# fabrizioromanelli/ORBSLAM2

Hardware: AMD Instinct MI355X
Metric: frames/sec ORB extract+match, KITTI 1241×376 stereo, 2000 feats; 1/2/4/8 GPU (higher is better)
Workload: dtype u8; 1 GPU; Stereo-KITTI00-02 1241x376, 2000 features, 8 levels: extract L+R + ComputeStereoMatches (64 pairs per step per GPU, weak scaling); distinct_pairs=16, chains_in_flight=1, stream_groups=1, quadtree_kernel=3, parallelism=frame-pair sharding, no data-path collective

## Files before the change

### orbslam2_amd/csrc/orbfe_api.hip

```cpp
#include "orbfe_host.h"

#include <algorithm>
#include <chrono>
#include <cmath>
#include <cstdarg>
#include <cstdio>
#include <cstdlib>
#include <cstring>
#include <new>
#include <vector>

static const int8_t k_bit_pattern_31[1024] = {
#include "orb_pattern_31.inc"
};
static thread_local char g_err[512] = "";

int orbfe_fail(orbfe_context *ctx, int code, const char *fmt, ...)
{
    char msg[512];
    va_list ap;
    va_start(ap, fmt);
    vsnprintf(msg, sizeof(msg), fmt, ap);
    va_end(ap);
    snprintf(g_err, sizeof(g_err), "%s", msg);
// ... 161 lines not shown
    T(&b.tail_plan, P.tail_plan, "pyramid tail plan");
    T(&b.pair_plan, P.pair_plan, "pyramid pair plan");
    T(&b.rs_tab, P.rs_tab, "resize table");
    T(&b.cell_aux, P.cell_aux, "cell table");
    T(&b.fast_lane_tab, P.fast_lane_tab, "cell table");
    T(&b.cell_info, P.cell_info, "cell table");
    T(&b.bk_tab, P.bk_tab, "bucket table");
    T(&b.bk_off, P.bk_off, "bucket partial table");
    T(&b.bk_emap, P.bk_emap, "bucket partial table");
    A(b.bk_part, B * P.bk_emap.size());
    T(&b.blur_tile_info, P.blur_tile_info, "blur tile table");
    T(&b.slot_level, P.slot_level, "slot table");
    T(&b.patch_uv, P.patch_uv, "patch table");
    T(&b.mom_tab, P.mom_tab, "moment table");
    uint32_t *d_pat = nullptr;
    A(d_pat, 256);
    if (rc == ORBFE_OK && hipMemcpy(d_pat, k_bit_pattern_31, 1024, hipMemcpyHostToDevice) != hipSuccess) rc = orbfe_fail(ctx, ORBFE_ERR_HIP, "pattern upload failed");
    b.pattern = d_pat;
    memcpy(ctx->pattern, k_bit_pattern_31, 1024);
    b.lv0 = b.pyr + c.lv[0].pyr_off; b.lv0_stride = c.pyr_bytes; b.lv0_pitch = c.lv[0].pitch; b.lv0_packed = 0;
    Z(b.proc_xy, B * c.sel_total * sizeof(uint32_t)); Z(b.proc_meta, B * c.sel_total * sizeof(uint32_t));
    Z(b.dbg_ts, 4096 * sizeof(long long)); Z(b.row_cnt, pairs * (size_t)p.height * sizeof(int));
    Z(b.bk_part, B * P.bk_emap.size() * sizeof(uint32_t));
    Z(b.kp_cnt, sizeof(int) * B); Z(b.sel_cnt, sizeof(int) * B * c.nlevels); Z(b.status, sizeof(int) * B);
    if (rc != ORBFE_OK) { orbfe_destroy(ctx); return rc; }
    *out = ctx;
    return ORBFE_OK;
} ORBFE_CATCH(nullptr)

extern "C" void orbfe_destroy(orbfe_context *ctx)
{
    if (!ctx) return;
    if (ctx->stream) { hipStreamSynchronize(ctx->stream); }
    for (void *q : ctx->allocs) hipFree(q);
    for (hipEvent_t e : ctx->events) hipEventDestroy(e);
    for (int g = 0; g < ORBFE_MAX_GROUPS; g++) {
        if (ctx->gstreams[g]) { hipStreamSynchronize(ctx->gstreams[g]); hipStreamDestroy(ctx->gstreams[g]); }
        if (ctx->ev_join[g]) hipEventDestroy(ctx->ev_join[g]);
    }
    if (ctx->ev_fork) hipEventDestroy(ctx->ev_fork);
    if (ctx->ev_latest) hipEventDestroy(ctx->ev_latest);
    if (ctx->ev_pack) { if (ctx->ev_pack_set) hipEventSynchronize(ctx->ev_pack); hipEventDestroy(ctx->ev_pack); }
    if (ctx->match) orbfe_match_state_destroy(ctx->match);
    if (ctx->match_device) orbfe_match_device_state_destroy(ctx->match_device);
    if (ctx->bow) orbfe_bow_state_destroy(ctx->bow);
    if (ctx->pose) orbfe_pose_state_destroy(ctx->pose);
    if (ctx->d_depth_in) hipFree(ctx->d_depth_in);
    if (ctx->h_in) hipHostFree(ctx->h_in);
    if (ctx->h_depth_in) hipHostFree(ctx->h_depth_in);
    if (ctx->h_out) hipHostFree(ctx->h_out);
    for (int sd = 0; sd < 2; sd++) { if (ctx->cfg.rm_xy[sd]) hipFree((void *)ctx->cfg.rm_xy[sd]); if (ctx->cfg.rm_a[sd]) hipFree((void *)ctx->cfg.rm_a[sd]); }
    if (ctx->stream) hipStreamDestroy(ctx->stream);
    delete ctx;
}

extern "C" int orbfe_get_camera(const orbfe_context *ctx, float *cam)
try {
    if (!ctx || !cam) return ORBFE_ERR_INVALID;
    cam[0] = ctx->params.fx; cam[1] = ctx->params.fy; cam[2] = ctx->params.cx; cam[3] = ctx->params.cy; cam[4] = ctx->params.bf;
    return ORBFE_OK;
} ORBFE_CATCH(nullptr)

static int wait_latest(orbfe_context *ctx);
extern "C" int orbfe_set_pattern(orbfe_context *ctx, const int32_t *pattern)
try {
    ORBFE_ENTRY(ctx);
// ... 125 lines not shown
    const size_t i = (size_t)img0;
    o.pyr += i * c.pyr_bytes; o.blur += i * c.blur_bytes;
    o.lv0 = o.pyr + c.lv[0].pyr_off; o.lv0_stride = c.pyr_bytes; o.lv0_pitch = c.lv[0].pitch; o.lv0_packed = 0;
    o.cell_cnt += i * c.cells_total; o.cell_base += i * c.cells_total;
    o.cell_xy += i * c.cells_total * c.cell_cap; o.cell_sc += i * c.cells_total * c.cell_cap;
    o.cand_xy += i * c.cand_total; o.cand_sc += i * c.cand_total;
    o.idx0 += i * c.cand_total; o.idx1 += i * c.cand_total; o.ot_xy2 += i * c.cand_total;
    o.lvl_ncand += i * c.nlevels; o.sel_cnt += i * c.nlevels;
    o.bk_part += i * c.bk_part_total; o.bk_end += i * c.nlevels * 4097;
    if (o.ot3_scratch) o.ot3_scratch += i * c.nlevels * orbfe_octree3_node_bytes(c.max_nodes, orbfe_sort_cap(c.max_nodes));
    if (o.bk_best) o.bk_best += i * c.nlevels * ORBFE_BK_PYR;
    if (o.otg_scratch) o.otg_scratch += i * orbfe_otg_level_off(c, c.nlevels);
    o.sel_xy += i * c.sel_total; o.sel_sc += i * c.sel_total; o.proc_xy += i * c.sel_total; o.proc_meta += i * c.sel_total;
    o.kps = (KeyPointPOD *)o.kps + i * c.sel_total; o.desc += i * c.sel_total * 32;
    o.kp_cnt += i; o.status += i;
    o.u_right += i * c.sel_total; o.depth += i * c.sel_total; o.sad += i * c.sel_total;
    o.row_cnt += (i / 2) * (size_t)c.height; o.row_ent += (i / 2) * (size_t)c.height * c.row_cap;
    return o;
}

static int blur_ride_from_of(const orbfe_context *ctx, int n_images)
{
    if (!ctx->plan.fuse_blur) return ctx->cfg.nlevels;
    return n_images >= ctx->plan.blur_ride_min_images ? (ctx->plan.blur_ride_from < ctx->cfg.nlevels ? ctx->plan.blur_ride_from : ctx->cfg.nlevels) : ORBFE_MAX_LEVELS;
}

extern "C" int orbfe_blur_ride_from(const orbfe_context *ctx, int n_images)
try {
    if (!ctx) return ORBFE_ERR_INVALID;
    const int r = blur_ride_from_of(ctx, n_images);
    return r < ctx->cfg.nlevels ? r : (ctx->plan.fuse_blur && n_images < ctx->plan.blur_ride_min_images ? ctx->cfg.nlevels - 1 : ctx->cfg.nlevels);
} ORBFE_CATCH(nullptr)

static void run_chain(orbfe_context *ctx, const uint8_t *d_images, int img0, int n_images, int n_pairs, hipStream_t s, int group)
{
    const DeviceConfig &cfg = ctx->cfg;
    DeviceBuffers buf = shift_buffers(ctx->buf, cfg, img0);
    const uint8_t *src = d_images + (size_t)img0 * cfg.in_image_bytes;
    prof_mark(ctx, group, 0, s);
    if (ctx->plan.inplace_ok && cfg.in_cn == 1 && !cfg.rm_on) {
        buf.lv0 = src; buf.lv0_stride = cfg.in_image_bytes; buf.lv0_pitch = cfg.width; buf.lv0_packed = 1;
    } else {
        orbfe_launch_ingest(cfg, buf, src, n_images, s);
    }
    prof_mark(ctx, group, 1, s);
    const int ride_from = blur_ride_from_of(ctx, n_images);
    const int blurred = orbfe_launch_pyramid(cfg, buf, n_images, ctx->plan.fuse_blur, s, ride_from);
    prof_mark(ctx, group, 2, s);
    if (!ctx->plan.fuse_blur) orbfe_launch_blur(cfg, buf, n_images, blurred, s);
    prof_mark(ctx, group, 3, s);
    orbfe_launch_fast(cfg, buf, n_images, ctx->plan.use_octree3, s, ctx->plan.fuse_blur ? blurred : cfg.nlevels);
    prof_mark(ctx, group, 4, s);
    if (ctx->plan.use_octree3) orbfe_launch_octree3(cfg, buf, n_images, ctx->plan.ot_sort_cap, ctx->plan.ot3_lds, ctx->plan.ot3_nodes_in_hbm, s);
    else if (const hipError_t e = orbfe_launch_octree_generic(cfg, buf, n_images, ctx->plan.otg_nodes_in_hbm, s)) ctx->chain_err = e;
#ifdef ORBFE_PROFILE_CUTS
    {
        extern void orbfe_launch_dbg_sort_sel(const DeviceConfig &, const DeviceBuffers &, int, int, hipStream_t);
        static const int dbg_sort = getenv("ORBFE_DBG_SORT_SEL") ? atoi(getenv("ORBFE_DBG_SORT_SEL")) : 0;
        if (dbg_sort) orbfe_launch_dbg_sort_sel(cfg, buf, n_images, dbg_sort, s);
    }
#endif
    prof_mark(ctx, group, 5, s);
    orbfe_launch_describe(cfg, buf, n_images, n_pairs > 0, s);
    prof_mark(ctx, group, 6, s);
    if (n_pairs > 0) {
        if (cfg.half_patch != 15) orbfe_launch_stereo_rowlists(cfg, buf, n_pairs, s);
        orbfe_launch_stereo_match(cfg, buf, n_pairs, s);
        prof_mark(ctx, group, 7, s);
        orbfe_launch_stereo_median(cfg, buf, n_pairs, s);
        prof_mark(ctx, group, 8, s);
    }
}

static int enqueue_batch(orbfe_context *ctx, const uint8_t *d_images, int n_units, int imgs_per_unit, void *stream)
{
    hipStream_t s;
    if (const int rc = orbfe_enqueue_on(ctx, stream, false, &s)) return rc;
    ctx->prof_now = ctx->profiling && (ctx->prof_seq++ % (unsigned)ctx->prof_every) == 0;
    const int n_images = n_units * imgs_per_unit;
    int G = ctx->groups < n_units ? ctx->groups : n_units;
    if (G < 1) G = 1;
    if (G == 1) {
        run_chain(ctx, d_images, 0, n_images, imgs_per_unit == 2 ? n_units : 0, s, 0);
    } else {
        ORBFE_HIP_TRY(ctx, hipEventRecord(ctx->ev_fork, s));
        int u0 = 0;
        for (int g = 0; g < G; g++) {
            const int nu = n_units / G + (g < n_units % G ? 1 : 0);
            hipStream_t sg = ctx->gstreams[g];
            ORBFE_HIP_TRY(ctx, hipStreamWaitEvent(sg, ctx->ev_fork, 0));
            run_chain(ctx, d_images, u0 * imgs_per_unit, nu * imgs_per_unit, imgs_per_unit == 2 ? nu : 0, sg, g);
            ORBFE_HIP_TRY(ctx, hipEventRecord(ctx->ev_join[g], sg));
            ORBFE_HIP_TRY(ctx, hipStreamWaitEvent(s, ctx->ev_join[g], 0));
            u0 += nu;
        }
    }
    if (ctx->chain_err != hipSuccess) { const hipError_t e = ctx->chain_err; ctx->chain_err = hipSuccess; return orbfe_fail(ctx, ORBFE_ERR_HIP, "quadtree launch: %s", hipGetErrorString(e)); }
    ORBFE_HIP_TRY(ctx, hipGetLastError());
    ctx->last_src = (ctx->plan.inplace_ok && ctx->cfg.in_cn == 1 && !ctx->cfg.rm_on) ? d_images : nullptr;
    ctx->last_src_owned = ctx->last_src && ctx->last_src == ctx->d_in;
    ctx->last_images = n_images;
    ctx->epoch++;
    ctx->prof_groups = G;
    ctx->latest_foreign = s != ctx->stream;
    if (ctx->latest_foreign) ORBFE_HIP_TRY(ctx, hipEventRecord(ctx->ev_latest, s));
    if (ctx->prof_now) ctx->prof_calls++;
    return ORBFE_OK;
}

extern "C" int orbfe_quadtree_kernel(const orbfe_context *ctx)
try {
    if (!ctx) return 0;
    return ctx->plan.use_octree3 ? 3 : 1;
} ORBFE_CATCH(nullptr)

extern "C" int orbfe_quadtree_plan(const orbfe_context *ctx)
try {
    if (!ctx) return ORBFE_ERR_INVALID;
    if (ctx->plan.use_octree3) return ctx->plan.ot3_nodes_in_hbm ? 1 : 0;
    return ctx->plan.otg_nodes_in_hbm ? 3 : 2;
} ORBFE_CATCH(nullptr)

extern "C" int orbfe_set_streams(orbfe_context *ctx, int groups)
try {
    ORBFE_ENTRY(ctx);
    if (!ctx || groups < 1 || groups > ORBFE_MAX_GROUPS) return orbfe_fail(ctx, ORBFE_ERR_INVALID, "groups must be in [1, %d]", ORBFE_MAX_GROUPS);
    if (ctx->profiling) return orbfe_fail(ctx, ORBFE_ERR_INVALID, "change the stream count before enabling profiling");
    ORBFE_HIP_TRY(ctx, hipSetDevice(ctx->params.device));
    if (!ctx->ev_fork) ORBFE_HIP_TRY(ctx, hipEventCreateWithFlags(&ctx->ev_fork, hipEventDisableTiming));
    for (int g = 0; g < groups; g++) {
// ... 608 lines not shown
        return orbfe_fail(ctx, ORBFE_ERR_INVALID, "bad argument");
    { const int rcw = wait_latest(ctx); if (rcw != ORBFE_OK) return rcw; }
    const LevelInfo &L = ctx->cfg.lv[level];
    if (dst_stride < (size_t)L.w) return orbfe_fail(ctx, ORBFE_ERR_INVALID, "dst_stride smaller than level width");
    if (blurred) {
        const size_t bytes = (size_t)L.blur_tx * ((L.h + 3) / 4) * 128;
        std::vector<uint8_t> t(bytes);
        ORBFE_HIP_TRY(ctx, hipMemcpy(t.data(), ctx->buf.blur + (size_t)image * ctx->cfg.blur_bytes + L.blur_off, bytes, hipMemcpyDeviceToHost));
        for (int y = 0; y < L.h; y++)
            for (int x = 0; x < L.w; x += 4) {
                const size_t off = ((size_t)(y >> 2) * L.blur_tx + (x >> 5)) * 128 + (size_t)((x & 31) >> 2) * 16 + (size_t)(y & 3) * 4;
                memcpy(dst + (size_t)y * dst_stride + x, t.data() + off, (size_t)std::min(4, L.w - x));
            }
        return ORBFE_OK;
    }
    if (level == 0 && !blurred && ctx->last_src) {
        if (!ctx->last_src_owned && !ctx->input_retained)
            return orbfe_fail(ctx, ORBFE_ERR_UNSUPPORTED, "level 0 of the latest call is the caller's own image buffer (read in place, never copied): "
                                                    "call orbfe_set_input_retained(ctx, 1) if that buffer is still valid, or read the images there");
        ORBFE_HIP_TRY(ctx, hipMemcpy2D(dst, dst_stride, ctx->last_src + (size_t)image * ctx->cfg.in_image_bytes, (size_t)L.w, (size_t)L.w, (size_t)L.h, hipMemcpyDeviceToHost));
        return ORBFE_OK;
    }
    const uint8_t *src = ctx->buf.pyr + (size_t)image * ctx->cfg.pyr_bytes + L.pyr_off;
    ORBFE_HIP_TRY(ctx, hipMemcpy2D(dst, dst_stride, src, (size_t)L.pitch, (size_t)L.w, (size_t)L.h, hipMemcpyDeviceToHost));
    return ORBFE_OK;
} ORBFE_CATCH(ctx)

extern "C" int orbfe_fetch_candidates(orbfe_context *ctx, int image, int level, int32_t *xs, int32_t *ys,
                                      int32_t *scores, int cap, int *n)
try {
    ORBFE_ENTRY(ctx);
    if (!ctx || !n || image < 0 || image >= ctx->params.max_images || level < 0 || level >= ctx->cfg.nlevels)
        return orbfe_fail(ctx, ORBFE_ERR_INVALID, "bad argument");
    { const int rcw = wait_latest(ctx); if (rcw != ORBFE_OK) return rcw; }
    const DeviceConfig &c = ctx->cfg;
    const LevelInfo &L = c.lv[level];
    if (ctx->plan.use_octree3) {
        orbfe_launch_candidates_gather(c, ctx->buf, ctx->params.max_images, ctx->stream);
        ORBFE_HIP_TRY(ctx, hipStreamSynchronize(ctx->stream));
    }
    int nc = 0;
    ORBFE_HIP_TRY(ctx, hipMemcpy(&nc, ctx->buf.lvl_ncand + (size_t)image * c.nlevels + level, sizeof(int), hipMemcpyDeviceToHost));
    *n = nc;
    if (nc > cap) return orbfe_fail(ctx, ORBFE_ERR_CAPACITY, "caller buffers hold %d candidates, level has %d", cap, nc);
    if (nc == 0) return ORBFE_OK;
    std::vector<uint32_t> xy(nc);
    std::vector<uint8_t> sc(nc);
    ORBFE_HIP_TRY(ctx, hipMemcpy(xy.data(), ctx->buf.cand_xy + (size_t)image * c.cand_total + L.cand_off, sizeof(uint32_t) * nc, hipMemcpyDeviceToHost));
    ORBFE_HIP_TRY(ctx, hipMemcpy(sc.data(), ctx->buf.cand_sc + (size_t)image * c.cand_total + L.cand_off, (size_t)nc, hipMemcpyDeviceToHost));
    for (int i = 0; i < nc; i++) {
        if (xs) xs[i] = (int32_t)(xy[i] & 0xffffu);
        if (ys) ys[i] = (int32_t)(xy[i] >> 16);
        if (scores) scores[i] = sc[i];
    }
    return ORBFE_OK;
} ORBFE_CATCH(ctx)
```

### orbslam2_amd/csrc/orbfe_config.h

```cpp
#pragma once

#include <math.h>
#include <stddef.h>
#include <stdint.h>

#ifdef __HIPCC__
#define ORBFE_HD __attribute__((host, device)) inline __attribute__((always_inline))
#else
#define ORBFE_HD inline
#endif

#define ORBFE_MAX_LEVELS 16
#define ORBFE_TAIL_MAX 3
#define ORBFE_TAIL_COLS 64
#ifndef ORBFE_BLUR_ROWS
#define ORBFE_BLUR_ROWS 32
#endif
#define ORBFE_WAVE 64
#define PYR_MX 4
#define PYR_MY 3
#ifndef ORBFE_PYR_RB
#define ORBFE_PYR_RB 4
#endif
struct LevelInfo {
// ... 31 lines not shown
    int width, height;
    int edge_threshold, min_border;
    int ini_th, min_th;
    uint32_t ini_th_h2, min_th_h2;
    int half_patch;
    int cell_cap;
    int cells_total;
    int cand_total;
    int sel_total;
    int blur_tiles_total;
    int proc_order;
    int fast_blur_t0;
    uint32_t xcd_magic;
    int max_nodes;
    int bk_part_total;
    int row_cap;
    int patch_n;
    int tail_first, tail_n, tail_strips;
    int pp_max_images;
    int tail_max_images;
    int tail_src_words;
    int tail_words[ORBFE_TAIL_MAX];
    int tail_lds_y[ORBFE_TAIL_MAX];
    int tail_lds_buf[ORBFE_TAIL_MAX];
    int tail_lds_src, tail_lds_bytes;
    int umax[64];
    int taps[7];
    size_t pyr_bytes;
    size_t blur_bytes;
    float bf, fx, mb;
    int in_cn, in_coef[3], in_shift;
    size_t in_image_bytes;
    int rm_on, rm_sw, rm_sh;
    const uint32_t *rm_xy[2];
    const uint16_t *rm_a[2];
    int n_dist;
    float dist[5];
    float cam[4];
    LevelInfo lv[ORBFE_MAX_LEVELS];
};
static_assert(sizeof(LevelInfo) == 224 && sizeof(DeviceConfig) == 4168, "LevelInfo / DeviceConfig layout changed");
static_assert(offsetof(DeviceConfig, pyr_bytes) == 440 && offsetof(DeviceConfig, rm_xy) == 512 && offsetof(DeviceConfig, lv) == 584,
              "DeviceConfig layout changed");

#define ORBFE_BK_DEPTH 5
#define ORBFE_BK_BUCKETS 4096
#define ORBFE_BK_PYR 5460
#define ORBFE_BK_REF_MASK 0xffffffu
#define ORBFE_BK_KEY(sc, cell, slot) (((sc) << 24) | (ORBFE_BK_REF_MASK - (unsigned)(((cell) << 12) | (slot))))
#define ORBFE_BK_PART(cnt, key) ((cnt) | (((key) & 0xfffu) << 12) | ((key) & 0xff000000u))
#define ORBFE_BK_PART_KEY(e, cell) (((e) & 0xff000000u) | ((4095u - (unsigned)(cell)) << 12) | (((e) >> 12) & 0xfffu))

#define OT3_ROOTS 4
#define OT3_PYR (OT3_ROOTS * 1365)
#define OT3_HI (OT3_ROOTS * 85)

ORBFE_HD int resize_first_source(int dx, double scale, int src_w)
{
    const float fx = (float)(((double)dx + 0.5) * scale - 0.5);
    int sx = (int)floorf(fx);
    sx = sx < 0 ? 0 : sx;
    return sx >= src_w - 1 ? src_w - 1 : sx;
}
ORBFE_HD int resize_word_base(int xw, int dst_w, double scale, int src_w)
{
    int lo = 0x7fffffff;
    for (int j = 0; j < 4; j++) {
        int q = 4 * xw + j - PYR_MX;
        if (dst_w == 1) q = 0;
        else while (q < 0 || q >= dst_w) q = q < 0 ? -q : 2 * dst_w - 2 - q;
        lo = q < lo ? q : lo;
    }
    return resize_first_source(lo, scale, src_w);
}

static inline int max_cell_w(const DeviceConfig &cfg) { int m = 0; for (int l = 0; l < cfg.nlevels; l++) m = cfg.lv[l].w_cell > m ? cfg.lv[l].w_cell : m; return m; }
// ... 42 lines not shown
```

### orbslam2_amd/csrc/orbfe_device.h

```cpp
#pragma once

#include <hip/hip_runtime.h>
#include <stdint.h>
#include <stdlib.h>

#include "orbfe_config.h"

typedef unsigned long long u64;

#ifdef ORBFE_PROFILE_CUTS
#define ORBFE_CUT_PARAM , int dbg
template <int N> __device__ __forceinline__ bool orbfe_phase_end() { asm volatile("; ORBFE_PHASE_END %0" ::"n"(N)); return true; }
#define ORBFE_CUT(n) (orbfe_phase_end<n>() && dbg == (n))
#define ORBFE_CUT_ARG(env) , orbfe_cut_value(env)
static inline int orbfe_cut_value(const char *env) { const char *v = getenv(env); return v ? atoi(v) : 0; }
#else
#define ORBFE_CUT_PARAM
#define ORBFE_CUT(n) false
#define ORBFE_CUT_ARG(env)
#endif

struct DeviceBuffers {
    uint8_t *pyr;
    const uint8_t *lv0;
// ... 26 lines not shown
    int *sad;
    int *status;
    int *row_cnt;
    uint2 *row_ent;
    const uint32_t *bk_tab;
    const uint32_t *bk_emap;
    const uint32_t *bk_off;
    const uint32_t *rs_tab;
    const uint4 *cell_info;
    const uint2 *cell_aux;
    const uint32_t *fast_lane_tab;
    const uint32_t *blur_tile_info;
    const uint32_t *rs_blk;
    const int *pair_plan;
    const int *tail_plan;
    long long *dbg_ts;
    const uint8_t *slot_level;
    const int16_t *patch_uv;
    const uint32_t *mom_tab;
    const uint32_t *pattern;
    uint8_t *otg_scratch;
};

struct KeyPointPOD {
    float x, y, size, angle, response;
    int32_t octave, class_id;
};
static_assert(sizeof(KeyPointPOD) == 28, "keypoint must match cv::KeyPoint");

void orbfe_launch_ingest(const DeviceConfig &cfg, const DeviceBuffers &buf, const uint8_t *d_images,
                         int n_images, hipStream_t s);
int orbfe_launch_pyramid(const DeviceConfig &cfg, const DeviceBuffers &buf, int n_images, bool fuse_blur, hipStream_t s, int ride_from = ORBFE_MAX_LEVELS);
void orbfe_launch_blur(const DeviceConfig &cfg, const DeviceBuffers &buf, int n_images, int first_level, hipStream_t s);
void orbfe_launch_fast(const DeviceConfig &cfg, const DeviceBuffers &buf, int n_images, bool buckets, hipStream_t s, int blur_first_level);
hipError_t orbfe_launch_octree_generic(const DeviceConfig &cfg, const DeviceBuffers &buf, int n_images, bool nodes_in_hbm, hipStream_t s);
int orbfe_octree_generic_prepare(const DeviceConfig &cfg, bool nodes_in_hbm);
void orbfe_launch_octree3(const DeviceConfig &cfg, const DeviceBuffers &buf, int n_images, int sort_cap, size_t lds, bool nodes_in_hbm, hipStream_t s);
void orbfe_launch_candidates_gather(const DeviceConfig &cfg, const DeviceBuffers &buf, int n_images, hipStream_t s);
int orbfe_octree3_prepare(size_t lds, bool nodes_in_hbm);
void orbfe_launch_describe(const DeviceConfig &cfg, const DeviceBuffers &buf, int n_images, bool stereo, hipStream_t s);
void orbfe_launch_stereo_rowlists(const DeviceConfig &cfg, const DeviceBuffers &buf, int n_pairs, hipStream_t s);
void orbfe_launch_stereo_match(const DeviceConfig &cfg, const DeviceBuffers &buf, int n_pairs, hipStream_t s);
void orbfe_launch_stereo_median(const DeviceConfig &cfg, const DeviceBuffers &buf, int n_pairs, hipStream_t s);
void orbfe_launch_rgbd(const DeviceConfig &cfg, const DeviceBuffers &buf, const float *d_depth,
                       size_t depth_pitch_floats, int image, hipStream_t s);
void orbfe_launch_undistort(const DeviceConfig &cfg, const void *d_keys_in, void *d_keys_out, int n, hipStream_t s);
struct GridFrame;
void orbfe_launch_grid_build(const GridFrame &f, hipStream_t s);
struct orbfe_context;
struct orbfe_grid_keyframe;
int orbfe_grid_frame_of_record(orbfe_context *ctx, const orbfe_grid_keyframe *kf, GridFrame &f);
void orbfe_launch_rgbd_u16(const DeviceConfig &cfg, const DeviceBuffers &buf, const uint16_t *d_depth, size_t depth_pitch_px,
                           float factor, int image, hipStream_t s);
void orbfe_launch_rgbd_batch(const DeviceConfig &cfg, const DeviceBuffers &buf, const void *d_depth, bool is_u16, float factor, int n_images, hipStream_t s);
struct PackedOffsets { size_t counts, level_counts, xy, angle, response, desc, u_right, depth; };
void orbfe_launch_pack_results(const DeviceConfig &cfg, const DeviceBuffers &buf, uint8_t *d_out, const PackedOffsets &lay, int n_out, int img_step, bool stereo, hipStream_t s);
```

### orbslam2_amd/csrc/orbfe_fast.hip

```cpp
#include "orbfe_common.hpp"
#include "orbfe_blur_wave.hpp"

__device__ __forceinline__ int fast_score16(const uint8_t *t, int pitch, int minth)
{
    const int v = t[0];
    int d[16];
    d[0] = v - t[3 * pitch];       d[1] = v - t[3 * pitch + 1];   d[2] = v - t[2 * pitch + 2];   d[3] = v - t[pitch + 3];
    d[4] = v - t[3];               d[5] = v - t[-pitch + 3];      d[6] = v - t[-2 * pitch + 2];  d[7] = v - t[-3 * pitch + 1];
    d[8] = v - t[-3 * pitch];      d[9] = v - t[-3 * pitch - 1];  d[10] = v - t[-2 * pitch - 2]; d[11] = v - t[-pitch - 3];
    d[12] = v - t[-3];             d[13] = v - t[pitch - 3];      d[14] = v - t[2 * pitch - 2];  d[15] = v - t[3 * pitch - 1];
    int mn2[16], mx2[16], mn4[16], mx4[16];
#pragma unroll
    for (int k = 0; k < 16; k++) { mn2[k] = min(d[k], d[(k + 1) & 15]); mx2[k] = max(d[k], d[(k + 1) & 15]); }
#pragma unroll
    for (int k = 0; k < 16; k++) { mn4[k] = min(mn2[k], mn2[(k + 2) & 15]); mx4[k] = max(mx2[k], mx2[(k + 2) & 15]); }
    int a = -512, b = 512;
#pragma unroll
    for (int k = 0; k < 16; k++) {
        const int mn9 = min(min(mn4[k], mn4[(k + 4) & 15]), d[(k + 8) & 15]);
        const int mx9 = max(max(mx4[k], mx4[(k + 4) & 15]), d[(k + 8) & 15]);
        a = max(a, mn9);
        b = min(b, mx9);
    }
    return max(minth, max(a, -b)) - 1;
// ... 26 lines not shown
    int r;
    unsigned long long c;
    asm("v_addc_co_u32_e64 %0, %1, %2, 0, %3" : "=v"(r), "=s"(c) : "v"(x), "s"(m));
    return r;
}

__device__ __forceinline__ unsigned long long neg_lo16(unsigned v) { unsigned long long m; asm("v_cmp_gt_i16_e64 %0, 0, %1" : "=s"(m) : "v"(v)); return m; }
__device__ __forceinline__ unsigned long long neg_hi16(unsigned v) { unsigned long long m; asm("v_cmp_gt_i32_e64 %0, 0, %1" : "=s"(m) : "v"(v)); return m; }
__device__ __forceinline__ unsigned lds_addr(const void *p) { return (unsigned)(unsigned long)(__attribute__((address_space(3))) const void *)p; }
__device__ __forceinline__ void lds_store_lo16(unsigned long long m, unsigned addr, unsigned v)
{
    unsigned long long save;
    asm volatile("s_and_saveexec_b64 %0, %1\n\tds_write_b16 %2, %3\n\ts_or_b64 exec, exec, %0" : "=&s"(save) : "s"(m), "v"(addr), "v"(v) : "memory", "scc");
}
__device__ __forceinline__ void lds_store_hi16(unsigned long long m, unsigned addr, unsigned v)
{
    unsigned long long save;
    asm volatile("s_and_saveexec_b64 %0, %1\n\tds_write_b16_d16_hi %2, %3\n\ts_or_b64 exec, exec, %0" : "=&s"(save) : "s"(m), "v"(addr), "v"(v) : "memory", "scc");
}

__device__ __forceinline__ unsigned h2min(unsigned a, unsigned b) { unsigned d; asm("v_pk_min_f16 %0, %1, %2" : "=v"(d) : "v"(a), "v"(b)); return d; }
__device__ __forceinline__ unsigned h2max(unsigned a, unsigned b) { unsigned d; asm("v_pk_max_f16 %0, %1, %2" : "=v"(d) : "v"(a), "v"(b)); return d; }
__device__ __forceinline__ unsigned h2min3(unsigned a, unsigned b, unsigned c) { unsigned d; asm("v_pk_minimum3_f16 %0, %1, %2, %3" : "=v"(d) : "v"(a), "v"(b), "v"(c)); return d; }
__device__ __forceinline__ unsigned h2max3(unsigned a, unsigned b, unsigned c) { unsigned d; asm("v_pk_maximum3_f16 %0, %1, %2, %3" : "=v"(d) : "v"(a), "v"(b), "v"(c)); return d; }
__device__ __forceinline__ unsigned h2add(unsigned a, unsigned b) { unsigned d; asm("v_pk_add_f16 %0, %1, %2" : "=v"(d) : "v"(a), "v"(b)); return d; }
__device__ __forceinline__ unsigned h2sub(unsigned a, unsigned b) { unsigned d; asm("v_pk_add_f16 %0, %1, %2 neg_lo:[0,1] neg_hi:[0,1]" : "=v"(d) : "v"(a), "v"(b)); return d; }

#define FAST_WAVE_SYNC() do { __builtin_amdgcn_s_waitcnt(0xc07f); __builtin_amdgcn_wave_barrier(); } while (0)
template <int TP, bool BK>
__global__ __launch_bounds__(256) __attribute__((amdgpu_waves_per_eu(6, 8))) void fast_cell_kernel(DeviceConfig cfg, DeviceBuffers buf, int n_images, int tile_pitch_rt, int tile_bytes, int sc_bytes, int q_bytes, int lds_per_wave ORBFE_CUT_PARAM)
{
    const int tile_pitch = TP ? TP : tile_pitch_rt;
    extern __shared__ __attribute__((aligned(16))) uint8_t s_mem_all[];
    const int bpi_cells = (cfg.cells_total + 3) >> 2;
    const int bpi = bpi_cells + ((cfg.blur_tiles_total - cfg.fast_blur_t0 + 3) >> 2);
    int img, blk;
    if (!xcd_map_magic(bpi, n_images, cfg.xcd_magic, img, blk)) return;
    const int wave = __builtin_amdgcn_readfirstlane((int)(threadIdx.x >> 6));
    if (__builtin_expect(blk >= bpi_cells, 0)) {
        const int u = cfg.fast_blur_t0 + (blk - bpi_cells) * 4 + wave;
        if (u < cfg.blur_tiles_total) blur_wave(cfg, buf, img, u);
        return;
    }
    const int cell = blk * 4 + wave;
    if (cell >= cfg.cells_total) return;
    uint8_t *s_mem = s_mem_all + wave * lds_per_wave;
    const uint4 cinfo = const_load_u32x4(buf.cell_info + cell);
    const uint32_t aux_g = const_load_u32((const uint32_t *)buf.cell_aux + 2 * cell), aux_c = const_load_u32((const uint32_t *)buf.cell_aux + 2 * cell + 1);
    const uint32_t *lane_tab = buf.fast_lane_tab + ((aux_g & 0x1ffffu) << 9);
    const uint4 lt_a = *(const uint4 *)(lane_tab + ((threadIdx.x & 63) << 3));
    const uint2 lt_b = *(const uint2 *)(lane_tab + ((threadIdx.x & 63) << 3) + 4);
    const int level = (int)(cinfo.x & 0xffu);
    const LevelInfo &L = cfg.lv[level];
    const int ci = (int)cinfo.w;
    const int lane = threadIdx.x & 63;
    int *cnt_out = buf.cell_cnt + (size_t)img * cfg.cells_total + cell;
    if (!(cinfo.x & 0x100u)) {
        if (lane == 0) *cnt_out = 0;
        return;
    }
    const int ini_x = (int)(cinfo.y & 0xffffu), ini_y = (int)(cinfo.y >> 16);
    const int max_x = ini_x + (int)(cinfo.z & 0xffu);
    const int tw = (int)(cinfo.z & 0xffu), th = (int)((cinfo.z >> 8) & 0xffu);
    const int iw = tw - 6, ih = th - 6;
    const int cell_x0 = ini_x - cfg.min_border, cell_y0 = ini_y - cfg.min_border;
    unsigned tabx = 0u, taby = 0u, bk_off = ~0u;
    if (BK) {
        bk_off = const_load_u32(buf.bk_off + cell);
        const uint32_t *bx_tab = buf.bk_tab + L.bk_xoff + 3 + cell_x0;
        const uint32_t *by_tab = buf.bk_tab + L.bk_yoff + 3 + cell_y0;
        tabx = *(const uint32_t *)((const uint8_t *)bx_tab + min((unsigned)lane << 2, (unsigned)(iw - 1) << 2));
        taby = *(const uint32_t *)((const uint8_t *)by_tab + min((unsigned)lane << 2, (unsigned)(ih - 1) << 2));
    }
    uint8_t *s_tile = s_mem;
    uint8_t *s_sc = s_mem + tile_bytes;
    uint16_t *s_q1 = (uint16_t *)(s_sc + sc_bytes);
    uint16_t *s_q2 = s_q1;
    uint8_t *s_qf = s_tile;
// ... 221 lines not shown
    }
    FAST_WAVE_SYNC();
    const int n_out = run < cfg.cell_cap ? run : cfg.cell_cap;
    for (int p0 = 0; p0 < n_out; p0 += 64) {
        const int pos = p0 + lane;
        const bool v = pos < n_out;
        const unsigned rc = v ? (s_q2[pos] & 0x7fffu) : 0u;
        const int r = (int)(rc >> 8) - 1, c = rc & 255;
        unsigned tx = 0u, ty = 0u;
        if (part) { tx = (unsigned)__shfl((int)tabx, c, 64); ty = (unsigned)__shfl((int)taby, r, 64); }
        if (v) {
            const unsigned x = (unsigned)(c + 3 + cell_x0);
            const unsigned y = (unsigned)(r + 3 + cell_y0);
            const unsigned sc = s_sc[(r + 1) * scp + c + 1];
            oxy[pos] = x | (y << 16);
            osc[pos] = (uint8_t)sc;
            if (part) {
                const int li = ((int)(ty >> 16) - by0) * ncols + ((int)(tx >> 16) - gx0);
                atomicAdd(&s_ac[li], 1u);
                atomicMax(&s_ab[li], ORBFE_BK_KEY(sc, (unsigned)ci, (unsigned)pos));
            }
        }
    }
    if (lane == 0) *cnt_out = run < cfg.cell_cap ? run : cfg.cell_cap;
    if (part && !ORBFE_CUT(5)) {
        FAST_WAVE_SYNC();
        if (lane < nb) buf.bk_part[(size_t)img * cfg.bk_part_total + bk_off + lane] = ORBFE_BK_PART(s_ac[lane], s_ab[lane]);
    }
}


static inline int max_cell_h(const DeviceConfig &cfg) { int m = 0; for (int l = 0; l < cfg.nlevels; l++) m = cfg.lv[l].h_cell > m ? cfg.lv[l].h_cell : m; return m; }

void orbfe_launch_fast(const DeviceConfig &cfg_in, const DeviceBuffers &buf, int n_images, bool buckets, hipStream_t s, int blur_first_level)
{
    DeviceConfig cfg = cfg_in;
    cfg.fast_blur_t0 = blur_first_level < cfg.nlevels ? cfg.lv[blur_first_level].blur_tile_off : cfg.blur_tiles_total;
    const int mw = max_cell_w(cfg), mh = max_cell_h(cfg);
    const int tile_pitch = orbfe_fast_tile_pitch(cfg);
    const int tile_rows = mh + 6;
    const int tile_bytes = (tile_pitch * tile_rows + 15) & ~15;
    const int sc_bytes = ((mw + 2) * (mh + 2) + 15) & ~15;
    const int q_bytes = (2 * mw * mh + 15) & ~15;
    const int tile_region = tile_bytes > mw * mh ? tile_bytes : ((mw * mh + 15) & ~15);
    const int lds_per_wave = tile_region + sc_bytes + q_bytes + 512;
    const size_t lds = (size_t)4 * lds_per_wave;
    const int bpi = (cfg.cells_total + 3) / 4 + (cfg.blur_tiles_total - cfg.fast_blur_t0 + 3) / 4;
    cfg.xcd_magic = xcd_map_magic_host(bpi, n_images);
    dim3 grid(xcd_grid(bpi, n_images));
#define FAST_LAUNCH(TP)                                                                                                                   \
    do {                                                                                                                              \
        if (buckets) hipLaunchKernelGGL((fast_cell_kernel<TP, true>), grid, dim3(256), lds, s, cfg, buf, n_images, tile_pitch, tile_region, sc_bytes, q_bytes, lds_per_wave ORBFE_CUT_ARG("ORBFE_FAST_DBG")); \
        else hipLaunchKernelGGL((fast_cell_kernel<TP, false>), grid, dim3(256), lds, s, cfg, buf, n_images, tile_pitch, tile_region, sc_bytes, q_bytes, lds_per_wave ORBFE_CUT_ARG("ORBFE_FAST_DBG")); \
    } while (0)
    switch (tile_pitch) {
    case 32: FAST_LAUNCH(32); break;
    case 48: FAST_LAUNCH(48); break;
    case 64: FAST_LAUNCH(64); break;
    default: FAST_LAUNCH(0); break;
    }
#undef FAST_LAUNCH
}
```

### orbslam2_amd/csrc/orbfe_host.h

```cpp
#pragma once
#include <hip/hip_runtime.h>
#include <mutex>
#include <vector>
#include "../../include/orbfe.h"
#include "orbfe_device.h"
#include "orbfe_plan.h"

struct DevBuf {
    void *p = nullptr;
    size_t bytes = 0;
    int ensure(size_t need)
    {
        if (need <= bytes) return 0;
        if (p) (void)hipFree(p);
        p = nullptr; bytes = 0;
        if (hipMalloc(&p, need) != hipSuccess) return -1;
        bytes = need;
        return 0;
    }
    DevBuf() = default;
    DevBuf(const DevBuf &) = delete;
    DevBuf &operator=(const DevBuf &) = delete;
    ~DevBuf() { if (p) (void)hipFree(p); }
};
// ... 20 lines not shown
    uint8_t *d_in = nullptr;
    float *d_depth_in = nullptr;
    uint8_t *h_in = nullptr;
    float *h_depth_in = nullptr;
    uint8_t *h_out = nullptr;
    DevBuf d_pack;
    hipEvent_t ev_pack = nullptr;
    bool ev_pack_set = false;
    DevBuf d_ham;
    DevBuf d_und;
    int last_images = 0;
    unsigned epoch = 0;
    std::vector<int> slot_cnt;
    unsigned slot_cnt_epoch = ~0u;
    LaunchPlan plan;
    const uint8_t *last_src = nullptr;
    bool last_src_owned = false;
    bool input_retained = false;
    bool profiling = false;
    int prof_every = 1;
    unsigned prof_seq = 0;
    bool prof_now = false;
    int prof_only = -1;
    std::vector<hipEvent_t> events;
    int prof_calls = 0;
    int prof_stages[64];
    int prof_groups = 1;
    hipEvent_t ev_latest = nullptr;
    bool latest_foreign = false;
    std::recursive_mutex mu;
    int groups = 1;
    hipStream_t gstreams[ORBFE_MAX_GROUPS] = {};
    hipEvent_t ev_fork = nullptr, ev_join[ORBFE_MAX_GROUPS] = {};
    int8_t pattern[1024];
    std::vector<void *> allocs;
    orbfe_match_state *match = nullptr;
    orbfe_match_device_state *match_device = nullptr;
    orbfe_bow_state *bow = nullptr;
    orbfe_pose_state *pose = nullptr;
    DevBuf init_scratch, init_sync;
    DevBuf recon_scratch, recon_sync;
    DevBuf sim3_opt_scratch, sim3_opt_sync;
    DevBuf sim3_ransac_scratch, sim3_ransac_sync;
    DevBuf pnp_ransac_scratch, pnp_ransac_sync;
    hipError_t chain_err = hipSuccess;
    char err[512];
};

int orbfe_fail(orbfe_context *ctx, int code, const char *fmt, ...);
#define ORBFE_HIP_TRY(ctx, expr) do { hipError_t e_ = (expr); if (e_ != hipSuccess) return orbfe_fail(ctx, ORBFE_ERR_HIP, "%s: %s", #expr, hipGetErrorString(e_)); } while (0)
#define ORBFE_ENTRY(ctx)                                  \
    std::unique_lock<std::recursive_mutex> orbfe_entry_lock_; \
    if (ctx) orbfe_entry_lock_ = std::unique_lock<std::recursive_mutex>((ctx)->mu)

int orbfe_ctx_slot_count(orbfe_context *ctx, int slot, int *cnt);
int orbfe_ctx_wait_foreign_stream(orbfe_context *ctx);
int orbfe_ctx_order_after_extraction(orbfe_context *ctx, hipStream_t s);
int orbfe_enqueue_on(orbfe_context *ctx, void *stream, bool after_extraction, hipStream_t *s);
orbfe_match_state *orbfe_ctx_match_state(orbfe_context *ctx);
orbfe_match_device_state *orbfe_ctx_match_device_state(orbfe_context *ctx);
orbfe_bow_state *orbfe_ctx_bow_state(orbfe_context *ctx);
orbfe_pose_state *orbfe_ctx_pose_state(orbfe_context *ctx);

#include <exception>
#include <new>
#define ORBFE_CATCH(ctxexpr)                                                                                              \
// ... 4 lines not shown
```

### orbslam2_amd/csrc/orbfe_plan.cpp

```cpp
#include "orbfe_plan.h"

#include <algorithm>
#include <climits>
#include <cmath>
#include <cstdarg>
#include <cstdio>
#include <cstdlib>
#include <cstring>

static int plan_fail(char *err, size_t err_len, int code, const char *fmt, ...)
{
    va_list ap;
    va_start(ap, fmt); vsnprintf(err, err_len, fmt, ap); va_end(ap);
    return code;
}

PlanKnobs PlanKnobs::from_env()
{
    PlanKnobs k;
    auto first = [](const char *name) { const char *v = getenv(name); return v ? v[0] : '\0'; };
    auto tri = [&](const char *name) { const char f = first(name); return f == '1' ? 1 : (f == '0' ? 0 : -1); };
    k.no_inplace = first("ORBFE_NO_INPLACE") == '1';
    k.no_pair = tri("ORBFE_NO_PAIR");
    k.no_tail = tri("ORBFE_NO_TAIL");
    k.pyr_lds = first("ORBFE_PYR_LDS") == '1';
    k.no_fuse = first("ORBFE_NO_FUSE") == '1';
    k.no_proc_order = first("ORBFE_NO_PROC_ORDER") == '1';
    { const char *v = getenv("ORBFE_OCTREE"); k.octree_generic = v && atoi(v) == 1; k.octree_generic_hbm = v && atoi(v) == 2; }
    { const char *v = getenv("ORBFE_BLUR_RIDE_FROM"); if (v && v[0] >= '0' && v[0] <= '9') k.blur_ride_from = atoi(v); }
    k.host_trace = getenv("ORBFE_HOST_TRACE") != nullptr;
    return k;
}

static void src_hull(const std::vector<uint32_t> &tab, int off, int i0, int i1, int &lo, int &hi)
{
    lo = INT_MAX; hi = -1;
    for (int i = i0; i < i1; i++) { const int a = (int)(tab[off + i] & 0xffffu), b = (int)(tab[off + i] >> 16); lo = std::min(lo, std::min(a, b)); hi = std::max(hi, std::max(a, b)); }
}

static int cv_round_f(float v) { return (int)lrintf(v); }

static void gaussian_taps_q8(int ksize, double sigma, int *taps)
{
    double g[64];
    double scale2x = -0.5 / (sigma * sigma);
    double sum = 0.0;
    for (int i = 0; i < ksize; i++) {
        double x = (double)i - (double)(ksize - 1) * 0.5;
        g[i] = exp(scale2x * x * x);
        sum += g[i];
    }
    sum = 1.0 / sum;
    for (int i = 0; i < ksize; i++) g[i] *= sum;
    int n2 = ksize / 2;
    double err = 0.0;
    long acc = 0;
    for (int i = 0; i < n2; i++) {
        double adj = g[i] * 256.0 + err;
        long v0 = lrint(adj);
        err = adj - (double)v0;
        taps[i] = (int)v0;
        taps[ksize - 1 - i] = (int)v0;
        acc += 2 * v0;
    }
// ... 540 lines not shown
        }
    }
    {
        std::vector<int16_t> uv;
        const int hp = p.half_patch_size;
        for (int v = -hp; v <= hp; v++) {
            const int d = c.umax[v < 0 ? -v : v];
            for (int u = -d; u <= d; u++) uv.push_back((int16_t)((u & 0xff) | ((v & 0xff) << 8)));
        }
        while (uv.size() % 64) uv.push_back(0);
        c.patch_n = (int)uv.size();
        P.patch_uv.swap(uv);
    }
    {
        std::vector<uint32_t> mt(12 * 64, 0u);
        if (p.half_patch_size == 15)
            for (int lane = 0; lane < 62; lane++) {
                const int r = lane >> 1, half = lane & 1, v = r - 15, um = c.umax[v < 0 ? -v : v];
                for (int k = 0; k < 4; k++) {
                    uint32_t wu = 0, w1 = 0;
                    for (int j = 0; j < 4; j++) {
                        const int u = 16 * half + 4 * k + j - 15;
                        if (u >= -um && u <= um) { wu |= (uint32_t)(u + 16) << (8 * j); w1 |= 1u << (8 * j); }
                    }
                    mt[(size_t)lane * 12 + k] = wu;
                    mt[(size_t)lane * 12 + 4 + k] = w1;
                }
                mt[(size_t)lane * 12 + 8] = (uint32_t)v;
            }
        P.mom_tab.swap(mt);
    }
    P.inplace_ok = !knobs.no_inplace && c.nlevels >= 2 && c.lv[1].rs_direct && c.tail_first != 1 && p.width >= 16 && p.height >= 8;
    if (knobs.host_trace) fprintf(stderr, "orbfe: level 0 of packed grey input: %s\n", P.inplace_ok ? "read in place (no ingest launch)" : "copied by ingest16_kernel");
    return ORBFE_OK;
}
```

### orbslam2_amd/csrc/orbfe_plan.h

```cpp
#pragma once

#include "../../include/orbfe.h"
#include "orbfe_config.h"

#include <vector>

struct PlanKnobs {
    bool no_inplace = false;
    int no_pair = -1;
    int no_tail = -1;
    bool pyr_lds = false;
    bool no_fuse = false;
    bool no_proc_order = false;
    bool octree_generic = false;
    bool octree_generic_hbm = false;
    int blur_ride_from = -1;
    bool host_trace = false;
    static PlanKnobs from_env();
};

struct LaunchPlan {
    float scale[ORBFE_MAX_LEVELS], inv_scale[ORBFE_MAX_LEVELS], sigma2[ORBFE_MAX_LEVELS], inv_sigma2[ORBFE_MAX_LEVELS];
    int32_t feats[ORBFE_MAX_LEVELS];
    bool use_octree3 = false;
    size_t ot3_lds = 0;
    bool ot3_nodes_in_hbm = false;
    int ot_sort_cap = 0;
    bool otg_nodes_in_hbm = false;
    size_t otg_scratch_bytes = 0;
    bool fuse_blur = true;
    int blur_ride_from = 0, blur_ride_min_images = 64;
    bool inplace_ok = false;
};

struct HostPlan : LaunchPlan {
    DeviceConfig cfg;
    std::vector<uint32_t> rs_tab, rs_blk;
    std::vector<int> tail_plan, pair_plan;
    std::vector<uint32_t> cell_info, cell_aux, fast_lane_tab, bk_tab, bk_off, bk_emap, blur_tile_info;
    std::vector<uint8_t> slot_level;
    std::vector<int16_t> patch_uv;
    std::vector<uint32_t> mom_tab;
};

int orbfe_build_plan(const orbfe_params &p, int max_images, const PlanKnobs &knobs, HostPlan *plan, char *err, size_t err_len);
```

Measured before the change: 104,000 frames/s (1 frame = 1 stereo pair).

## Run level-0 FAST on a low-priority side stream concurrent with pyramid build

Splits the FAST launch into two cell ranges. Level 0 cells, plus its blur tiles when blur rides from level 0, go on a new low-priority side stream that forks before the pyramid launches. The remaining levels run after the pyramid on the main stream, and the two streams join before the quadtree. This lets level-0 corner detection overlap the pyramid kernels, at the cost of extra events and stream handling and a range encoding in the kernel config. It is enabled by default only when a call has at least 64 images, with a single group and profiling off.

```diff
diff --git a/orbslam2_amd/csrc/orbfe_api.hip b/orbslam2_amd/csrc/orbfe_api.hip
--- a/orbslam2_amd/csrc/orbfe_api.hip
+++ b/orbslam2_amd/csrc/orbfe_api.hip
@@ -217,6 +217,9 @@
 {
     if (!ctx) return;
     if (ctx->stream) { hipStreamSynchronize(ctx->stream); }
+    if (ctx->side_stream) { hipStreamSynchronize(ctx->side_stream); hipStreamDestroy(ctx->side_stream); }
+    if (ctx->ev_side_fork) hipEventDestroy(ctx->ev_side_fork);
+    if (ctx->ev_side_join) hipEventDestroy(ctx->ev_side_join);
     for (void *q : ctx->allocs) hipFree(q);
     for (hipEvent_t e : ctx->events) hipEventDestroy(e);
     for (int g = 0; g < ORBFE_MAX_GROUPS; g++) {
@@ -408,6 +411,23 @@
     return r < ctx->cfg.nlevels ? r : (ctx->plan.fuse_blur && n_images < ctx->plan.blur_ride_min_images ? ctx->cfg.nlevels - 1 : ctx->cfg.nlevels);
 } ORBFE_CATCH(nullptr)
 
+static bool side_stream_ready(orbfe_context *ctx)
+{
+    if (ctx->side_stream) return true;
+    int least = 0, greatest = 0;
+    if (hipDeviceGetStreamPriorityRange(&least, &greatest) != hipSuccess) return false;
+    const int prio = least;
+    if (hipEventCreateWithFlags(&ctx->ev_side_fork, hipEventDisableTiming) != hipSuccess || hipEventCreateWithFlags(&ctx->ev_side_join, hipEventDisableTiming) != hipSuccess ||
+        hipStreamCreateWithPriority(&ctx->side_stream, hipStreamNonBlocking, prio) != hipSuccess) {
+        if (ctx->ev_side_fork) { hipEventDestroy(ctx->ev_side_fork); ctx->ev_side_fork = nullptr; }
+        if (ctx->ev_side_join) { hipEventDestroy(ctx->ev_side_join); ctx->ev_side_join = nullptr; }
+        ctx->side_stream = nullptr;
+        (void)hipGetLastError();
+        return false;
+    }
+    return true;
+}
+
 static void run_chain(orbfe_context *ctx, const uint8_t *d_images, int img0, int n_images, int n_pairs, hipStream_t s, int group)
 {
     const DeviceConfig &cfg = ctx->cfg;
@@ -421,11 +441,25 @@
     }
     prof_mark(ctx, group, 1, s);
     const int ride_from = blur_ride_from_of(ctx, n_images);
+    FastRange fr[2];
+    const bool side_blur = ctx->plan.fuse_blur && ride_from == 0;
+    bool split = n_images >= ctx->plan.fast_split_min_images && ctx->groups == 1 && !ctx->profiling &&
+                 orbfe_fast_launches(cfg, true, side_blur, cfg.nlevels, fr) == 2 && side_stream_ready(ctx);
+    if (ctx->plan.host_trace && ctx->fast_split_traced != (int)split) {
+        fprintf(stderr, "orbfe: FAST: %s\n", split ? "level 0 on the side stream beside the pyramid's launches, the other levels behind them" : "one launch");
+        ctx->fast_split_traced = (int)split;
+    }
+    if (split) {
+        if (hipEventRecord(ctx->ev_side_fork, s) != hipSuccess || hipStreamWaitEvent(ctx->side_stream, ctx->ev_side_fork, 0) != hipSuccess) { split = false; ctx->chain_err = hipErrorUnknown; }
+        else if (const hipError_t e = orbfe_launch_fast(cfg, buf, n_images, ctx->plan.use_octree3, ctx->side_stream, fr[0])) ctx->chain_err = e;
+    }
     const int blurred = orbfe_launch_pyramid(cfg, buf, n_images, ctx->plan.fuse_blur, s, ride_from);
     prof_mark(ctx, group, 2, s);
     if (!ctx->plan.fuse_blur) orbfe_launch_blur(cfg, buf, n_images, blurred, s);
     prof_mark(ctx, group, 3, s);
-    orbfe_launch_fast(cfg, buf, n_images, ctx->plan.use_octree3, s, ctx->plan.fuse_blur ? blurred : cfg.nlevels);
+    const int n_fast = orbfe_fast_launches(cfg, split, side_blur, ctx->plan.fuse_blur ? blurred : cfg.nlevels, fr);
+    if (const hipError_t e = orbfe_launch_fast(cfg, buf, n_images, ctx->plan.use_octree3, s, fr[n_fast - 1])) ctx->chain_err = e;
+    if (split && (hipEventRecord(ctx->ev_side_join, ctx->side_stream) != hipSuccess || hipStreamWaitEvent(s, ctx->ev_side_join, 0) != hipSuccess)) ctx->chain_err = hipErrorUnknown;
     prof_mark(ctx, group, 4, s);
     if (ctx->plan.use_octree3) orbfe_launch_octree3(cfg, buf, n_images, ctx->plan.ot_sort_cap, ctx->plan.ot3_lds, ctx->plan.ot3_nodes_in_hbm, s);
     else if (const hipError_t e = orbfe_launch_octree_generic(cfg, buf, n_images, ctx->plan.otg_nodes_in_hbm, s)) ctx->chain_err = e;
@@ -471,7 +505,7 @@
             u0 += nu;
         }
     }
-    if (ctx->chain_err != hipSuccess) { const hipError_t e = ctx->chain_err; ctx->chain_err = hipSuccess; return orbfe_fail(ctx, ORBFE_ERR_HIP, "quadtree launch: %s", hipGetErrorString(e)); }
+    if (ctx->chain_err != hipSuccess) { const hipError_t e = ctx->chain_err; ctx->chain_err = hipSuccess; return orbfe_fail(ctx, ORBFE_ERR_HIP, "launch refused: %s", hipGetErrorString(e)); }
     ORBFE_HIP_TRY(ctx, hipGetLastError());
     ctx->last_src = (ctx->plan.inplace_ok && ctx->cfg.in_cn == 1 && !ctx->cfg.rm_on) ? d_images : nullptr;
     ctx->last_src_owned = ctx->last_src && ctx->last_src == ctx->d_in;
@@ -1146,11 +1180,12 @@
     ORBFE_ENTRY(ctx);
     if (!ctx || !n || image < 0 || image >= ctx->params.max_images || level < 0 || level >= ctx->cfg.nlevels)
         return orbfe_fail(ctx, ORBFE_ERR_INVALID, "bad argument");
+    if (image >= ctx->last_images) return orbfe_fail(ctx, ORBFE_ERR_INVALID, "image %d: the latest extraction call filled %d image slots", image, ctx->last_images);
     { const int rcw = wait_latest(ctx); if (rcw != ORBFE_OK) return rcw; }
     const DeviceConfig &c = ctx->cfg;
     const LevelInfo &L = c.lv[level];
     if (ctx->plan.use_octree3) {
-        orbfe_launch_candidates_gather(c, ctx->buf, ctx->params.max_images, ctx->stream);
+        orbfe_launch_candidates_gather(c, ctx->buf, ctx->last_images, ctx->stream);
         ORBFE_HIP_TRY(ctx, hipStreamSynchronize(ctx->stream));
     }
     int nc = 0;
diff --git a/orbslam2_amd/csrc/orbfe_config.h b/orbslam2_amd/csrc/orbfe_config.h
--- a/orbslam2_amd/csrc/orbfe_config.h
+++ b/orbslam2_amd/csrc/orbfe_config.h
@@ -87,6 +87,7 @@
     int in_cn, in_coef[3], in_shift;
     size_t in_image_bytes;
     int rm_on, rm_sw, rm_sh;
+    int fast_cell_c0;
     const uint32_t *rm_xy[2];
     const uint16_t *rm_a[2];
     int n_dist;
@@ -97,6 +98,17 @@
 static_assert(sizeof(LevelInfo) == 224 && sizeof(DeviceConfig) == 4168, "LevelInfo / DeviceConfig layout changed");
 static_assert(offsetof(DeviceConfig, pyr_bytes) == 440 && offsetof(DeviceConfig, rm_xy) == 512 && offsetof(DeviceConfig, lv) == 584,
               "DeviceConfig layout changed");
+static_assert(offsetof(DeviceConfig, fast_cell_c0) == 508, "DeviceConfig layout changed");
+
+struct FastRange { int c0, c1, t0, t1; };
+ORBFE_HD void fast_range_decode(int v, int total, int &lo, int &hi) { lo = v < 0 ? 0 : v; hi = v < 0 ? -v : total; }
+static inline bool fast_range_encode(int lo, int hi, int total, int *v)
+{
+    if (lo >= hi) { *v = total; return true; }
+    if (hi == total) { *v = lo; return true; }
+    if (lo == 0) { *v = -hi; return true; }
+    return false;
+}
 
 #define ORBFE_BK_DEPTH 5
 #define ORBFE_BK_BUCKETS 4096
diff --git a/orbslam2_amd/csrc/orbfe_device.h b/orbslam2_amd/csrc/orbfe_device.h
--- a/orbslam2_amd/csrc/orbfe_device.h
+++ b/orbslam2_amd/csrc/orbfe_device.h
@@ -82,7 +82,7 @@
                          int n_images, hipStream_t s);
 int orbfe_launch_pyramid(const DeviceConfig &cfg, const DeviceBuffers &buf, int n_images, bool fuse_blur, hipStream_t s, int ride_from = ORBFE_MAX_LEVELS);
 void orbfe_launch_blur(const DeviceConfig &cfg, const DeviceBuffers &buf, int n_images, int first_level, hipStream_t s);
-void orbfe_launch_fast(const DeviceConfig &cfg, const DeviceBuffers &buf, int n_images, bool buckets, hipStream_t s, int blur_first_level);
+hipError_t orbfe_launch_fast(const DeviceConfig &cfg, const DeviceBuffers &buf, int n_images, bool buckets, hipStream_t s, const FastRange &r);
 hipError_t orbfe_launch_octree_generic(const DeviceConfig &cfg, const DeviceBuffers &buf, int n_images, bool nodes_in_hbm, hipStream_t s);
 int orbfe_octree_generic_prepare(const DeviceConfig &cfg, bool nodes_in_hbm);
 void orbfe_launch_octree3(const DeviceConfig &cfg, const DeviceBuffers &buf, int n_images, int sort_cap, size_t lds, bool nodes_in_hbm, hipStream_t s);
diff --git a/orbslam2_amd/csrc/orbfe_fast.hip b/orbslam2_amd/csrc/orbfe_fast.hip
--- a/orbslam2_amd/csrc/orbfe_fast.hip
+++ b/orbslam2_amd/csrc/orbfe_fast.hip
@@ -82,18 +82,21 @@
 {
     const int tile_pitch = TP ? TP : tile_pitch_rt;
     extern __shared__ __attribute__((aligned(16))) uint8_t s_mem_all[];
-    const int bpi_cells = (cfg.cells_total + 3) >> 2;
-    const int bpi = bpi_cells + ((cfg.blur_tiles_total - cfg.fast_blur_t0 + 3) >> 2);
+    int c0, c1, t0, t1;
+    fast_range_decode(cfg.fast_cell_c0, cfg.cells_total, c0, c1);
+    fast_range_decode(cfg.fast_blur_t0, cfg.blur_tiles_total, t0, t1);
+    const int bpi_cells = (c1 - c0 + 3) >> 2;
+    const int bpi = bpi_cells + ((t1 - t0 + 3) >> 2);
     int img, blk;
     if (!xcd_map_magic(bpi, n_images, cfg.xcd_magic, img, blk)) return;
     const int wave = __builtin_amdgcn_readfirstlane((int)(threadIdx.x >> 6));
     if (__builtin_expect(blk >= bpi_cells, 0)) {
-        const int u = cfg.fast_blur_t0 + (blk - bpi_cells) * 4 + wave;
-        if (u < cfg.blur_tiles_total) blur_wave(cfg, buf, img, u);
+        const int u = t0 + (blk - bpi_cells) * 4 + wave;
+        if (u < t1) blur_wave(cfg, buf, img, u);
         return;
     }
-    const int cell = blk * 4 + wave;
-    if (cell >= cfg.cells_total) return;
+    const int cell = c0 + blk * 4 + wave;
+    if (cell >= c1) return;
     uint8_t *s_mem = s_mem_all + wave * lds_per_wave;
     const uint4 cinfo = const_load_u32x4(buf.cell_info + cell);
     const uint32_t aux_g = const_load_u32((const uint32_t *)buf.cell_aux + 2 * cell), aux_c = const_load_u32((const uint32_t *)buf.cell_aux + 2 * cell + 1);
@@ -381,10 +384,12 @@
 
 static inline int max_cell_h(const DeviceConfig &cfg) { int m = 0; for (int l = 0; l < cfg.nlevels; l++) m = cfg.lv[l].h_cell > m ? cfg.lv[l].h_cell : m; return m; }
 
-void orbfe_launch_fast(const DeviceConfig &cfg_in, const DeviceBuffers &buf, int n_images, bool buckets, hipStream_t s, int blur_first_level)
+hipError_t orbfe_launch_fast(const DeviceConfig &cfg_in, const DeviceBuffers &buf, int n_images, bool buckets, hipStream_t s, const FastRange &r)
 {
     DeviceConfig cfg = cfg_in;
-    cfg.fast_blur_t0 = blur_first_level < cfg.nlevels ? cfg.lv[blur_first_level].blur_tile_off : cfg.blur_tiles_total;
+    if (!fast_range_encode(r.c0, r.c1, cfg.cells_total, &cfg.fast_cell_c0) || !fast_range_encode(r.t0, r.t1, cfg.blur_tiles_total, &cfg.fast_blur_t0)) return hipErrorInvalidValue;
+    const int n_cells = r.c1 > r.c0 ? r.c1 - r.c0 : 0, n_tiles = r.t1 > r.t0 ? r.t1 - r.t0 : 0;
+    if (n_cells + n_tiles == 0) return hipSuccess;
     const int mw = max_cell_w(cfg), mh = max_cell_h(cfg);
     const int tile_pitch = orbfe_fast_tile_pitch(cfg);
     const int tile_rows = mh + 6;
@@ -394,7 +399,7 @@
     const int tile_region = tile_bytes > mw * mh ? tile_bytes : ((mw * mh + 15) & ~15);
     const int lds_per_wave = tile_region + sc_bytes + q_bytes + 512;
     const size_t lds = (size_t)4 * lds_per_wave;
-    const int bpi = (cfg.cells_total + 3) / 4 + (cfg.blur_tiles_total - cfg.fast_blur_t0 + 3) / 4;
+    const int bpi = (n_cells + 3) / 4 + (n_tiles + 3) / 4;
     cfg.xcd_magic = xcd_map_magic_host(bpi, n_images);
     dim3 grid(xcd_grid(bpi, n_images));
 #define FAST_LAUNCH(TP)                                                                                                                   \
@@ -409,4 +414,5 @@
     default: FAST_LAUNCH(0); break;
     }
 #undef FAST_LAUNCH
-}
+    return hipSuccess;
+}
diff --git a/orbslam2_amd/csrc/orbfe_host.h b/orbslam2_amd/csrc/orbfe_host.h
--- a/orbslam2_amd/csrc/orbfe_host.h
+++ b/orbslam2_amd/csrc/orbfe_host.h
@@ -76,6 +76,9 @@
     int groups = 1;
     hipStream_t gstreams[ORBFE_MAX_GROUPS] = {};
     hipEvent_t ev_fork = nullptr, ev_join[ORBFE_MAX_GROUPS] = {};
+    hipStream_t side_stream = nullptr;
+    hipEvent_t ev_side_fork = nullptr, ev_side_join = nullptr;
+    int fast_split_traced = -1;
     int8_t pattern[1024];
     std::vector<void *> allocs;
     orbfe_match_state *match = nullptr;
diff --git a/orbslam2_amd/csrc/orbfe_plan.cpp b/orbslam2_amd/csrc/orbfe_plan.cpp
--- a/orbslam2_amd/csrc/orbfe_plan.cpp
+++ b/orbslam2_amd/csrc/orbfe_plan.cpp
@@ -28,8 +28,22 @@
     k.no_proc_order = first("ORBFE_NO_PROC_ORDER") == '1';
     { const char *v = getenv("ORBFE_OCTREE"); k.octree_generic = v && atoi(v) == 1; k.octree_generic_hbm = v && atoi(v) == 2; }
     { const char *v = getenv("ORBFE_BLUR_RIDE_FROM"); if (v && v[0] >= '0' && v[0] <= '9') k.blur_ride_from = atoi(v); }
+    k.fast_split = tri("ORBFE_FAST_SPLIT");
     k.host_trace = getenv("ORBFE_HOST_TRACE") != nullptr;
     return k;
+}
+
+int orbfe_fast_launches(const DeviceConfig &c, bool split, bool side_blur, int blur_first, FastRange out[2])
+{
+    auto tile_off = [&](int l) { return l < c.nlevels ? c.lv[l].blur_tile_off : c.blur_tiles_total; };
+    const int cut = c.nlevels >= 2 ? c.lv[1].cell_off : 0;
+    if (!split || cut <= 0 || cut >= c.cells_total) {
+        out[0] = FastRange{0, c.cells_total, tile_off(blur_first), c.blur_tiles_total};
+        return 1;
+    }
+    out[0] = FastRange{0, cut, 0, side_blur ? tile_off(1) : 0};
+    out[1] = FastRange{cut, c.cells_total, tile_off(side_blur && blur_first < 1 ? 1 : blur_first), c.blur_tiles_total};
+    return 2;
 }
 
 static void src_hull(const std::vector<uint32_t> &tab, int off, int i0, int i1, int &lo, int &hi)
@@ -636,5 +650,7 @@
     }
     P.inplace_ok = !knobs.no_inplace && c.nlevels >= 2 && c.lv[1].rs_direct && c.tail_first != 1 && p.width >= 16 && p.height >= 8;
     if (knobs.host_trace) fprintf(stderr, "orbfe: level 0 of packed grey input: %s\n", P.inplace_ok ? "read in place (no ingest launch)" : "copied by ingest16_kernel");
+    P.fast_split_min_images = p.nlevels < 2 || knobs.fast_split == 0 ? INT_MAX : (knobs.fast_split == 1 ? 1 : std::max(64, P.blur_ride_min_images));
+    P.host_trace = knobs.host_trace;
     return ORBFE_OK;
 }
diff --git a/orbslam2_amd/csrc/orbfe_plan.h b/orbslam2_amd/csrc/orbfe_plan.h
--- a/orbslam2_amd/csrc/orbfe_plan.h
+++ b/orbslam2_amd/csrc/orbfe_plan.h
@@ -15,6 +15,7 @@
     bool octree_generic = false;
     bool octree_generic_hbm = false;
     int blur_ride_from = -1;
+    int fast_split = -1;
     bool host_trace = false;
     static PlanKnobs from_env();
 };
@@ -31,7 +32,11 @@
     bool fuse_blur = true;
     int blur_ride_from = 0, blur_ride_min_images = 64;
     bool inplace_ok = false;
+    int fast_split_min_images = 0x7fffffff;
+    bool host_trace = false;
 };
+
+int orbfe_fast_launches(const DeviceConfig &cfg, bool split, bool side_blur, int blur_first, FastRange out[2]);
 
 struct HostPlan : LaunchPlan {
     DeviceConfig cfg;
```

After: 107,300 frames/s (1 frame = 1 stereo pair), median of 6. 1.03x the previous value.
